# CPJKU/beat_this

Hardware: AMD Instinct MI355X
Metric: audio-seconds processed/sec (higher is better)
Workload: dtype f32 activations, f16x3 products (3 x f16 MFMA on hi+lo operand halves, f32 accumulate); main-layer attention P.V: 2 x, probabilities as fp16 hi parts

## Files before the change

beat_this_amd/_lib.py:

```python
from __future__ import annotations

import ctypes as C
import os
import subprocess

import torch

PKG_DIR = os.path.dirname(os.path.abspath(__file__))
LIB_PATH = os.path.join(PKG_DIR, "libbeat_this_amd.so")
if os.environ.get("BT_DEV") == "1" and os.environ.get("BT_LIB_PATH"):
    LIB_PATH = os.environ["BT_LIB_PATH"]
SOURCES = ["gemm.hip", "gemm2.hip", "gemm3.hip", "gemm_mx8.hip", "attn.hip", "attn2.hip", "fused.hip", "fused2.hip", "qkv_front.hip", "frontend.hip", "logmel.hip",
           "tail.hip", "dbn.hip", "metrics.hip", "loss.hip", "data.hip", "train.hip", "optim.hip", "engine.hip"]
HEADERS = ["common.h", "chain.h", "kernels.h", "attn_x3_loop.inc", "attn_hq2_loop.inc", os.path.join("..", "..", "include", "beat_this_amd.h")]

BT_OK, BT_ERR_ARG, BT_ERR_HIP, BT_ERR_WORKSPACE = 0, -1, -2, -3
ABI_VERSION = 600
PREC_F32, PREC_HALF, PREC_F32X3 = 0, 1, 3
OPT_X3_ATTN_P16, OPT_X3_GEMM_FP8, OPT_WS_GUARD = 1, 2, 3
MAX_LAYERS = 32
PROFILE_CATEGORIES = ["stem", "qkv_gemm", "attn_flash", "out_gemm", "ff1_gemm", "ff2_gemm", "conv_gemm",
                      "linear_gemm", "head", "ff_fused", "attn_freq_fused", "layer_tail"]

GEMM_EPI_STORE, GEMM_EPI_RESID, GEMM_EPI_QKV = 0, 1, 2
GEMM_F_RMS, GEMM_F_BIAS, GEMM_F_GELU, GEMM_F_OUT_F32, GEMM_F_A_F32, GEMM_F_CONV, GEMM_F_ROWMAP = 1, 2, 4, 8, 16, 32, 64


class PairWeights(C.Structure):
    _fields_ = [("dim", C.c_int32), ("heads", C.c_int32), ("w_qkvg", C.c_void_p * 2), ("b_gates", C.c_void_p),
                ("w_out", C.c_void_p * 2), ("w_ff1", C.c_void_p * 2), ("b_ff1", C.c_void_p),
                ("w_ff2", C.c_void_p * 2), ("b_ff2", C.c_void_p),
                ("w_ff_frag", C.c_void_p * 2), ("w_qkv_frag", C.c_void_p),
                ("w_outff_frag", C.c_void_p * 2), ("w_attnff_frag", C.c_void_p * 2),
                ("w_tail_frag", C.c_void_p),
# ... 352 lines not shown
```

beat_this_amd/csrc/engine.hip:

```cpp
#include <algorithm>
#include <cmath>
#include <cstddef>
#include <cstdio>
#include <cstring>
#include <mutex>
#include <string>
#include <vector>

#include "../../include/beat_this_amd.h"
#include "common.h"
#include "kernels.h"


static thread_local std::string g_err;
static int bt_set_error(int code, const std::string& msg) {
  g_err = msg;
  return code;
}
int bt_set_error_external(int code, const char* msg) { return bt_set_error(code, msg); }

namespace prof {
struct Rec { int cat; hipEvent_t a, b; };
struct State { bool on = false; std::vector<Rec> recs; };
struct Scope {
// ... 9 lines not shown
};
}

struct FwdGraph { int B, T, prec; void* ws; hipGraphExec_t exec; unsigned long stamp; };

struct bt_engine {
  bt_model_desc d;
  prof::State prof;
  std::mutex mu;
  std::vector<FwdGraph> graphs;
  unsigned long graph_clock = 0;
  hipStream_t cap_stream = nullptr;
  std::vector<int> warm;
  int x3_attn_p16 = 1;
  int x3_gemm_fp8 = 0;
  int ws_guard = 0;
};
enum { CAT_STEM = 0, CAT_QKV, CAT_ATTN_FLASH, CAT_OUT, CAT_FF1, CAT_FF2, CAT_CONV, CAT_LINEAR,
       CAT_HEAD, CAT_FF_FUSED, CAT_ATTN_FREQ_FUSED, CAT_LAYER_TAIL, CAT_COUNT };

namespace {

inline size_t align_up(size_t v, size_t a) { return (v + a - 1) / a * a; }

struct Workspace {
  float* xa; float* xb; float* xm; float* gates; void* xmb;
  void* qkv; void* ao; void* hid;
  void* qf; void* kf; void* vf; float* gates_h; int nbp;
  float* ssq[2];
  int* status;
// ... 120 lines not shown
  bool qkv8;
  bool out8;
  bool ff8;
  bool next8;
  bool tail;
  bool shadow_dead;
};

enum { LAYERS_GENERIC, LAYERS_FRAG_HALF, LAYERS_FRAG_X3 };

struct Route {
  bool x3;
  int fp;
  int gp, wp;
  int x3_attn, x3_attn_front;
  bool half_shadow;
  int layers;
  struct Block { PairRoute freq, time; bool conv3; bool x_dead; } blk[3];
  bool lin3, lin_f8;
  struct Layer { PairRoute pair; FragLayer frag; } layer[BT_MAX_LAYERS];
};

#ifndef BT_SKIP_DEAD_STORES
#define BT_SKIP_DEAD_STORES 1
#endif
Route plan_route(const bt_engine& e, int B, int T, int prec, int first, int last, const Workspace& ws) {
  const bt_model_desc& d = e.d;
  const int D = d.transformer_dim;
  Route r;
  r.x3 = prec == BT_PREC_F32X3;
  r.fp = r.x3 ? BT_PREC_F32 : prec;
  r.gp = prec;
  r.wp = r.x3 ? BT_PREC_HALF : prec;
  r.x3_attn = r.x3 ? 4 | ((e.x3_attn_p16 == 1 || e.x3_attn_p16 == 2) ? BT_X3_P16 : 0) : 0;
  r.x3_attn_front = r.x3 ? 4 | (e.x3_attn_p16 >= 2 ? BT_X3_P16 : 0) : 0;
  auto pair = [&](const bt_pair_weights& w) {
    PairRoute p;
    p.ff_fused = w.dim <= 128 && w.w_ff_frag[r.fp];
    p.outff = p.ff_fused && w.w_outff_frag[r.fp] && w.w_attnff_frag[r.fp];
    p.split = r.x3 && w.w_outff_frag_x3 && w.w_attnff_frag_x3;
    p.time_frag = r.x3 ? p.outff && p.split && w.w_qkv_frag_x3 : p.ff_fused && r.fp == BT_PREC_HALF && w.w_qkv_frag;
    return p;
  };

  r.half_shadow = prec == BT_PREC_HALF && D >= 128 && D % 64 == 0;
  const long wide = (long)B * T * d.ff_mult * D;
  bool frag_x3 = r.x3 && D >= 128 && D % 128 == 0 && wide * 4 < 0x7fffffffL;
  for (int l = 0; frag_x3 && l < d.n_layers; ++l)
    frag_x3 = d.layers[l].w_qkvg_x3 && d.layers[l].w_out_x3 && d.layers[l].w_ff1_x3 && d.layers[l].w_ff2_x3;
  const bool frag_half = r.half_shadow && D % 128 == 0 && wide * 2 < 0x7fffffffL;
  r.layers = frag_x3 ? LAYERS_FRAG_X3 : frag_half ? LAYERS_FRAG_HALF : LAYERS_GENERIC;

  const bool lin3_fits = (frag_half || (frag_x3 && d.lin_w_x3)) && gemm3_supported(linear3_params(d, ws, B, T, frag_x3, false));
  for (int blk = 0; blk < 3; ++blk) {
    Route::Block& rb = r.blk[blk];
    rb.freq = pair(d.front[blk][0]);
    rb.time = pair(d.front[blk][1]);
    const Gemm3P cg = conv3_params(d, ws, blk, B, T, frag_x3, blk == 2 && lin3_fits);
    rb.conv3 = d.partial_transformers && rb.time.outff && (frag_x3 ? rb.time.split : frag_half) && cg.N >= 128 && cg.W &&
               gemm3_supported(cg);
    rb.x_dead = BT_SKIP_DEAD_STORES && rb.conv3 && frag_x3;
  }
  r.lin3 = lin3_fits && (!frag_x3 || r.blk[2].conv3);
  r.lin_f8 = r.lin3 && frag_x3 && e.x3_gemm_fp8 >= 2 && d.n_layers > 0 && d.layers[0].w_qkvg_f8;

  for (int l = 0; l < d.n_layers; ++l) {
    const bt_pair_weights& w = d.layers[l];
    FragLayer& f = r.layer[l].frag;
    r.layer[l].pair = pair(w);
    f.qkv8 = l == 0 ? first == 0 && r.lin_f8 : r.layer[l - 1].frag.next8;
    f.out8 = frag_x3 && e.x3_gemm_fp8 >= 2 && w.w_out_f8;
    f.ff8 = frag_x3 && e.x3_gemm_fp8 >= 1 && w.w_ff1_f8 && w.w_ff2_f8;
    f.next8 = frag_x3 && e.x3_gemm_fp8 >= 2 && l + 1 < d.n_layers && d.layers[l + 1].w_qkvg_f8 && w.w_ff2_f8;
    f.tail = frag_half && w.w_tail_frag && layer_tail_supported(D, d.ff_mult * D);
// ... 143 lines not shown
  AttnFragP a;
  memset(&a, 0, sizeof a);
  a.q = ws.qf; a.k = ws.kf; a.v = ws.vf; a.gates = ws.gates_h; a.out = ws.ao; a.heads = H; a.inner = D; a.nbp = ws.nbp;
  attn_rows(a, B, T, 1);
  a.x3 = r.x3_attn; a.out_f32 = f.out8 ? 2 : 0; a.status = status; a.fix_mask = ws.fix_mask;
  LAUNCH_CAT(CAT_ATTN_FLASH, s, launch_attn_frag(a, s), r.x3 ? "attention (hi + lo)" : "attention");
  if (f.tail) {
    LayerTailP t;
    t.x = ws.xm; t.M = M; t.C = D; t.hidden = HID; t.ao = ws.ao; t.wfrag = pw.w_tail_frag; t.b1 = pw.b_ff1; t.b2 = pw.b_ff2;
    t.xb = ws.xmb; t.ssq_out = ws.ssq[0];
    LAUNCH_CAT(CAT_LAYER_TAIL, s, launch_layer_tail(t, s), "layer tail (out-projection + feed-forward)");
    return BT_OK;
  }
  memset(&g, 0, sizeof g);
  g.A = ws.ao; g.lda = D; g.M = M; g.K = D; g.W = w(pw.w_out, pw.w_out_x3, pw.w_out_f8, f.out8); g.N = D; g.epi = G3_RESID;
  g.x3 = r.x3 | (f.out8 ? G3_X3_F8 : 0) | (f.ff8 ? G3_X3_OUT_F8 : 0); g.status = status;
  g.x = ws.xm; g.ldx = D; g.xb = ws.xmb; g.ssq_out = ws.ssq[1];
  LAUNCH_CAT(CAT_OUT, s, launch_gemm3(g, s), r.x3 ? "out-proj gemm (hi + lo)" : "out-proj gemm");
  memset(&g, 0, sizeof g);
  g.A = ws.xmb; g.lda = D; g.M = M; g.K = D; g.W = w(pw.w_ff1, pw.w_ff1_x3, pw.w_ff1_f8, f.ff8); g.N = HID; g.epi = G3_FF1;
  g.x3 = r.x3 | (f.ff8 ? G3_X3_F8 | G3_X3_OUT_F8 : 0); g.status = status;
  g.bias = pw.b_ff1; g.ssq_in = ws.ssq[1]; g.ssq_parts = parts; g.out = ws.hid; g.ldo = HID;
  LAUNCH_CAT(CAT_FF1, s, launch_gemm3(g, s), r.x3 ? "ff1 gemm (hi + lo)" : "ff1 gemm");
  memset(&g, 0, sizeof g);
  g.A = ws.hid; g.lda = HID; g.M = M; g.K = HID; g.W = w(pw.w_ff2, pw.w_ff2_x3, pw.w_ff2_f8, f.ff8); g.N = D; g.epi = G3_RESID;
  g.x3 = r.x3 | (f.ff8 ? G3_X3_F8 : 0) | (f.next8 ? G3_X3_OUT_F8 : 0); g.status = status;
  g.bias = pw.b_ff2; g.x = ws.xm; g.ldx = D; g.xb = f.shadow_dead ? nullptr : ws.xmb; g.ssq_out = f.shadow_dead ? nullptr : ws.ssq[0];
  LAUNCH_CAT(CAT_FF2, s, launch_gemm3(g, s), r.x3 ? "ff2 gemm (hi + lo)" : "ff2 gemm");
  return BT_OK;
}

int frontend(prof::State* pf, const bt_model_desc& d, const Route& r, const float* spect, const Workspace& ws, int B, int T,
             hipStream_t s) {
  const StemP sp = stem_params(d, spect, front_x(ws, 0), B, T);
  LAUNCH_CAT(CAT_STEM, s, launch_stem(sp, s), "stem");
  for (int blk = 0; blk < 3; ++blk) {
    const Route::Block& rb = r.blk[blk];
    float* x = front_x(ws, blk);
    if (d.partial_transformers) {
      if (int rc = freq_half(pf, d.front[blk][0], rb.freq, r, d.rope, x, B, T, 32 >> blk, s)) return rc;
      if (int rc = time_half(pf, d.front[blk][1], rb.time, r, d.rope, x, ws, B, T, 32 >> blk, rb.conv3 ? ws.hid : nullptr, rb.x_dead, s))
        return rc;
    }
    if (rb.conv3) {
      const Gemm3P g = conv3_params(d, ws, blk, B, T, r.layers == LAYERS_FRAG_X3, blk == 2 && r.lin3);
      LAUNCH_CAT(CAT_CONV, s, launch_gemm3(g, s), "frontend conv gemm");
    } else {
      const GemmP g = conv_params(d, blk, r.wp, x, front_x(ws, blk + 1), B, T, !(blk == 2 && r.lin3));
      LAUNCH_CAT(CAT_CONV, s, launch_gemm(g, r.gp, s), "frontend conv gemm");
    }
  }
  if (r.lin3) {
    const Gemm3P g = linear3_params(d, ws, B, T, r.layers == LAYERS_FRAG_X3, r.lin_f8);
    LAUNCH_CAT(CAT_LINEAR, s, launch_gemm3(g, s), "frontend linear gemm");
    return BT_OK;
  }
  const GemmP g = linear_params(d, r.wp, front_x(ws, 3), ws.xm, r.half_shadow ? ws.xmb : nullptr,
                                r.layers == LAYERS_FRAG_HALF ? ws.ssq[0] : nullptr, B, T);
  LAUNCH_CAT(CAT_LINEAR, s, launch_gemm(g, r.gp, s), "frontend linear gemm");
  if (r.layers == LAYERS_FRAG_X3)
    LAUNCH_CAT(CAT_LINEAR, s, launch_shadow_ssq(ws.xm, ws.xmb, ws.ssq[0], (long)B * T, d.transformer_dim, s, 1), "hl32 shadow of the residual stream");
  return BT_OK;
}

}

extern "C" {

// ... 25 lines not shown
  e->warm.clear();
}
void bt_engine_destroy(bt_engine* e) {
  if (!e) return;
  for (auto& r : e->prof.recs) { (void)hipEventDestroy(r.a); (void)hipEventDestroy(r.b); }
  drop_graphs(e);
  if (e->cap_stream) (void)hipStreamDestroy(e->cap_stream);
  delete e;
}

int bt_engine_set_option(bt_engine* e, int option, int value) {
  if (!e) return bt_set_error(BT_ERR_ARG, "null argument");
  std::lock_guard<std::mutex> lock(e->mu);
  if (option == BT_OPT_X3_ATTN_P16 && value >= 0 && value <= 3) { if (e->x3_attn_p16 != value) drop_graphs(e); e->x3_attn_p16 = value; return BT_OK; }
  if (option == BT_OPT_X3_GEMM_FP8 && value >= 0 && value <= 2) { if (e->x3_gemm_fp8 != value) drop_graphs(e); e->x3_gemm_fp8 = value; return BT_OK; }
  if (option == BT_OPT_WS_GUARD && value >= 0 && value % 256 == 0) { if (e->ws_guard != value) drop_graphs(e); e->ws_guard = value; return BT_OK; }
  return bt_set_error(BT_ERR_ARG, "unknown engine option / value");
}
int bt_engine_get_option(const bt_engine* e, int option, int* value) {
  if (!e || !value) return bt_set_error(BT_ERR_ARG, "null argument");
  if (option == BT_OPT_X3_ATTN_P16) { *value = e->x3_attn_p16; return BT_OK; }
  if (option == BT_OPT_X3_GEMM_FP8) { *value = e->x3_gemm_fp8; return BT_OK; }
  if (option == BT_OPT_WS_GUARD) { *value = e->ws_guard; return BT_OK; }
  return bt_set_error(BT_ERR_ARG, "unknown engine option");
}

size_t bt_workspace_bytes(const bt_engine* e, int B, int T, int prec) {
  if (!e || B <= 0 || T <= 0) return 0;
  return carve(nullptr, B, T, e->d.transformer_dim, e->d.ff_mult, prec, (size_t)e->ws_guard).total;
}

int bt_workspace_regions(const bt_engine* e, int B, int T, int prec, int64_t* begin_end, int max) {
  if (!e || B <= 0 || T <= 0 || max < 0 || (max > 0 && !begin_end)) return bt_set_error(BT_ERR_ARG, "bad argument to bt_workspace_regions");
  if (prec != BT_PREC_F32 && prec != BT_PREC_HALF && prec != BT_PREC_F32X3) return bt_set_error(BT_ERR_ARG, "unknown precision");
  std::vector<int64_t> r;
  carve(nullptr, B, T, e->d.transformer_dim, e->d.ff_mult, prec, (size_t)e->ws_guard, &r);
  const int n = (int)(r.size() / 2);
// ... 565 lines not shown
```

beat_this_amd/csrc/fused2.hip:

```cpp
#include <cstdlib>
#include <type_traits>

#include "chain.h"
#include "kernels.h"

namespace {


typedef __amdgpu_buffer_rsrc_t rsrc_t;
typedef __attribute__((address_space(3))) void* lptr_t;
DEVI unsigned pk2_hf(float a, float b) {
  const hfx2 t = {(hf)a, (hf)b};
  return __builtin_bit_cast(unsigned, t);
}

#ifdef BT_DEV
__device__ long long* g_f2_dbg = nullptr;
#define F2_DBG g_f2_dbg
#define F2_ABL(p) ((p).abl)
#else
#define F2_DBG ((long long*)nullptr)
#define F2_ABL(p) 0
#endif

// ... 321 lines not shown
  const long long t_ff = dbg ? clock64() : 0;
  ff_tail<T, C>(ws, 1 + 2 * H, xn, b1s, p.b2, xrow, nullptr, ok, lane, g);
  if (dbg && lane == 0) {
    long long* d = dbg + ((long)blockIdx.x * 4 + wave) * 6;
    d[0] = t_ring - t_in; d[1] = t_ff - t_ring; d[2] = clock64() - t_ff; d[3] = ws.t_wait; d[4] = ws.t_bar; d[5] = 0;
  }
}

template <typename T>
int launch_outff_t(const FusedOutFFP& p, hipStream_t s) {
  dim3 grid((unsigned)((p.M + 127) / 128)), block(256);
  if constexpr (std::is_same<T, hl>::value) {
    if (p.shadow_only) {
      if (!p.xb) return -2;
      switch (p.C) {
        case 64: hipLaunchKernelGGL((outff_fused_kernel<T, 64, false>), grid, block, 0, s, p); break;
        case 128: hipLaunchKernelGGL((outff_fused_kernel<T, 128, false>), grid, block, 0, s, p); break;
        default: return -2;
      }
      return (int)hipGetLastError();
    }
  } else if (p.shadow_only) {
    return -2;
  }
  switch (p.C) {
    case 32: hipLaunchKernelGGL((outff_fused_kernel<T, 32>), grid, block, 0, s, p); break;
    case 64: hipLaunchKernelGGL((outff_fused_kernel<T, 64>), grid, block, 0, s, p); break;
    case 128: hipLaunchKernelGGL((outff_fused_kernel<T, 128>), grid, block, 0, s, p); break;
    default: return -2;
  }
// ... 39 lines not shown
```

beat_this_amd/csrc/gemm3.hip:

```cpp
#include <cstdlib>

#include "common.h"
#include "kernels.h"

struct G3CfgS { static constexpr int BM = 128, BN = 128, BK = 32, WGM = 2, WGN = 2, NST = 3, OCC = 3; };
struct G3CfgB { static constexpr int BM = 256, BN = 256, BK = 64, WGM = 2, WGN = 4, NST = 2, OCC = 1; };
struct G3CfgT { static constexpr int BM = 192, BN = 256, BK = 64, WGM = 2, WGN = 4, NST = 2, OCC = 1; };
struct G3CfgSX { static constexpr int BM = 128, BN = 128, BK = 64, WGM = 2, WGN = 2, NST = 2, OCC = 2; };
struct G3CfgBX { static constexpr int BM = 256, BN = 256, BK = 64, WGM = 2, WGN = 4, NST = 2, OCC = 1; };
struct G3CfgTX { static constexpr int BM = 192, BN = 256, BK = 64, WGM = 2, WGN = 4, NST = 2, OCC = 1; };
struct G3CfgMX { static constexpr int BM = 256, BN = 128, BK = 32, WGM = 2, WGN = 2, NST = 3, OCC = 2; };
struct G3CfgHX { static constexpr int BM = 64, BN = 128, BK = 64, WGM = 2, WGN = 2, NST = 3, OCC = 2; };

#ifndef X3_NSPLIT
#define X3_NSPLIT 2
#endif

namespace {

typedef G3CfgS CfgS;
typedef G3CfgB CfgB;

constexpr unsigned OOB = 0x80000000u;

#ifndef BT_NT_STORE
#define BT_NT_STORE 1
#endif
#if BT_NT_STORE
#define ST_STREAM(ptr, val) __builtin_nontemporal_store((val), (ptr))
#else
#define ST_STREAM(ptr, val) (*(ptr) = (val))
#endif

typedef __amdgpu_buffer_rsrc_t rsrc_t;
typedef __attribute__((address_space(3))) void* lptr_t;
typedef __attribute__((ext_vector_type(4))) unsigned int u32x4;
typedef __attribute__((ext_vector_type(2))) unsigned int u32x2;

DEVI unsigned pk2(float a, float b) {
  const hfx2 t = {(hf)a, (hf)b};
  return __builtin_bit_cast(unsigned, t);
// ... 531 lines not shown
    const int r4 = lane >> 4, cp = lane & 15;
    const unsigned ldx = (unsigned)p.ldx;
    const unsigned off_lane = (unsigned)(row0 + r4) * ldx + (unsigned)nb0;
    unsigned colq[4];
#pragma unroll
    for (int q = 0; q < 4; ++q) colq[q] = (unsigned)((cp ^ (4 * q + r4)) << 2);
    const int rows_left = p.M - row0 - r4;
    if (p.gelu) {
#pragma unroll
      for (int a = 0; a < FB; ++a)
#pragma unroll
        for (int b = 0; b < TB; ++b)
#pragma unroll
          for (int r = 0; r < 16; ++r) acc[a][b][r] = X3 ? gelu_erf(acc[a][b][r]) : gelu_tanh(acc[a][b][r]);
    }
#pragma unroll
    for (int b = 0; b < TB; ++b) {
      f32x4 xv[8];
#pragma unroll
      for (int ps = 0; ps < 8; ++ps) {
        const unsigned off = off_lane + (unsigned)(32 * b + 4 * ps) * ldx + colq[ps & 3];
        xv[ps] = (32 * b + 4 * ps < rows_left && !p.no_resid && p.x) ? *reinterpret_cast<const f32x4*>(p.x + off)
                                                               : f32x4{0.f, 0.f, 0.f, 0.f};
      }
#pragma unroll
      for (int a = 0; a < FB; ++a)
#pragma unroll
        for (int q = 0; q < 4; ++q)
          *reinterpret_cast<f32x4*>(wst + lr * 256 + (((8 * a + 2 * q + g) ^ (lr & 15)) << 4)) =
              f32x4{acc[a][b][4 * q], acc[a][b][4 * q + 1], acc[a][b][4 * q + 2], acc[a][b][4 * q + 3]};
#pragma unroll
      for (int ps = 0; ps < 8; ++ps) {
        const int r = ps * 4 + r4;
        const unsigned off = off_lane + (unsigned)(32 * b + 4 * ps) * ldx + colq[ps & 3];
        const bool ok = 32 * b + 4 * ps < rows_left;
        f32x4 v = *reinterpret_cast<const f32x4*>(wst + r * 256 + (cp << 4));
#pragma unroll
        for (int i = 0; i < 4; ++i) v[i] += xv[ps][i];
        if (ok) {
          if (p.x) *reinterpret_cast<f32x4*>(p.x + off) = v;
          if constexpr (X3) {
            if (xb) {
              const unsigned f = (unsigned)nb0 + colq[ps & 3];
              unsigned wh[2], wl[2];
              split2(v[0], v[1], wh[0], wl[0], amax);
              split2(v[2], v[3], wh[1], wl[1], amax);
              hf* d = xb + (2u * off - (f & 31u));
              *reinterpret_cast<u32x2*>(d) = u32x2{wh[0], wh[1]};
              if (p.x3 & G3_X3_OUT_F8) {
                char* gb = reinterpret_cast<char*>(d) - (f & 31u);
                *reinterpret_cast<unsigned*>(gb + 64) = pk4_f8(v[0], v[1], v[2], v[3]);
                *reinterpret_cast<unsigned*>(gb + 96) = lo4_f8(v[0], v[1], v[2], v[3], wh[0], wh[1]);
              } else {
                *reinterpret_cast<u32x2*>(d + 32) = u32x2{wl[0], wl[1]};
              }
            }
          } else {
            if (xb) *reinterpret_cast<u32x2*>(xb + off) = u32x2{pk2(v[0], v[1]), pk2(v[2], v[3])};
          }
        }
        if (p.ssq_out) {
          float ssq = ok ? fmaf(v[0], v[0], fmaf(v[1], v[1], fmaf(v[2], v[2], v[3] * v[3]))) : 0.f;
#pragma unroll
          for (int o = 8; o > 0; o >>= 1) ssq += __shfl_xor(ssq, o);
          if (ok && cp == 0) p.ssq_out[(unsigned)(n0 / 64 + wn) * (unsigned)p.M + (unsigned)(row0 + 32 * b + r)] = ssq;
        }
      }
    }
    }
  } else {
    constexpr int BLK_E = X3 ? 2048 : 1024;
    if (kind < 2) {
      hf* dst = reinterpret_cast<hf*>(kind == 0 ? p.qf : p.kf);
#pragma unroll
      for (int b = 0; b < TB; ++b) {
        if (tseq[b] >= p.n_seq) continue;
        const f32x4 (&cs)[4] = csv[b];
#pragma unroll
        for (int a = 0; a < FB; ++a) {
          const int head = (n0 - kind * p.inner + wn * 64 + a * 32) >> 5;
          hf* blk = dst + (((long)tseq[b] * p.heads + head) * p.nbp + tblk[b]) * BLK_E;
#pragma unroll
// ... 127 lines not shown
  const int force = (p.x3 & 15) == 2 ? 1 : (p.x3 & 15) == 3 ? 0 : force_big;
  const bool forced_small = (p.x3 & 15) == 4 || (p.x3 & 15) == 5;
  const long tiles192 = ((long)p.M + 191) / 192 * (p.N / 256);
  const bool fills = !p.x3 || tiles192 >= 160;
  const bool big = big_ok && !forced_small && (force == 1 || (force != 0 && p.epi == G3_RESID && p.K >= 1024 && p.M >= 4096 && fills) ||
                              (force != 0 && p.x3 && X3_BIG_FF1 && p.epi == G3_FF1 && p.M >= 4096));
  auto cost = [&](int bm) { const long t = ((long)p.M + bm - 1) / bm * (p.N / 256); return (t + 255) / 256 * bm; };
  const bool rows192 = big && p.epi == G3_RESID && force != 1 && cost(192) < cost(256);
  const long mx_tiles = ((long)p.M + 255) / 256 * ((p.N + 127) / 128);
  const bool f8 = (p.x3 & G3_X3_F8) != 0;
  const bool mx = p.x3 && !f8 && p.epi != G3_QKV && !big && !rows192 && force != 0 &&
                  ((p.x3 & 15) == 4 || (X3_MX && mx_tiles >= 512 && p.M >= 20000));
  const long sx_tiles = ((long)p.M + 127) / 128 * ((p.N + 127) / 128);
  const bool hx = p.x3 && p.epi == G3_RESID && !big && !rows192 && !mx &&
                  ((p.x3 & 15) == 5 || ((p.x3 & 15) <= 1 && force_big < 0 && (sx_tiles < 256 || (p.K < 1024 && p.M < 20000))));
  if (p.x3) {
#ifdef BT_DEV
    if (abl == 8 && p.epi == G3_FF1) { launch_cfg<G3_FF1, G3CfgSX, true, 8>(p, s); return (int)hipGetLastError(); }
    if (abl == 1 || abl == 4) {
      const bool b = big || rows192;
      if (p.epi == G3_FF1) { if (abl == 1) { if (b) launch_cfg<G3_FF1, G3CfgBX, true, 1>(p, s); else launch_cfg<G3_FF1, G3CfgSX, true, 1>(p, s); }
                             else { if (b) launch_cfg<G3_FF1, G3CfgBX, true, 4>(p, s); else launch_cfg<G3_FF1, G3CfgSX, true, 4>(p, s); } }
      else if (p.epi == G3_RESID) { if (abl == 1) { if (b) launch_cfg<G3_RESID, G3CfgBX, true, 1>(p, s); else launch_cfg<G3_RESID, G3CfgSX, true, 1>(p, s); }
                                    else { if (b) launch_cfg<G3_RESID, G3CfgBX, true, 4>(p, s); else launch_cfg<G3_RESID, G3CfgSX, true, 4>(p, s); } }
      else { if (abl == 1) launch_cfg<G3_QKV, G3CfgSX, true, 1>(p, s); else launch_cfg<G3_QKV, G3CfgSX, true, 4>(p, s); }
      return (int)hipGetLastError();
    }
#endif
    if (f8) {
      if (p.epi == G3_QKV) launch_cfg<G3_QKV, G3CfgSX, 2>(p, s);
      else if (p.epi == G3_FF1) { if (big) launch_cfg<G3_FF1, G3CfgBX, 2>(p, s); else launch_cfg<G3_FF1, G3CfgSX, 2>(p, s); }
      else if (hx) launch_cfg<G3_RESID, G3CfgHX, 2>(p, s);
      else if (rows192) launch_cfg<G3_RESID, G3CfgTX, 2>(p, s);
      else if (big) launch_cfg<G3_RESID, G3CfgBX, 2>(p, s);
      else launch_cfg<G3_RESID, G3CfgSX, 2>(p, s);
      return (int)hipGetLastError();
    }
    switch (p.epi) {
      case G3_FF1:
        if (mx) launch_cfg<G3_FF1, G3CfgMX, true>(p, s);
        else if (big) launch_cfg<G3_FF1, G3CfgBX, true>(p, s); else launch_cfg<G3_FF1, G3CfgSX, true>(p, s);
        break;
      case G3_RESID:
        if (mx) launch_cfg<G3_RESID, G3CfgMX, true>(p, s);
        else if (hx) launch_cfg<G3_RESID, G3CfgHX, true>(p, s);
        else if (rows192) launch_cfg<G3_RESID, G3CfgTX, true>(p, s);
        else if (big) launch_cfg<G3_RESID, G3CfgBX, true>(p, s);
        else launch_cfg<G3_RESID, G3CfgSX, true>(p, s);
        break;
      case G3_QKV: launch_cfg<G3_QKV, G3CfgSX, true>(p, s); break;
      default: return -1;
    }
    return (int)hipGetLastError();
  }
  switch (p.epi) {
    case G3_FF1:
      if (big) launch_cfg<G3_FF1, CfgB>(p, s);
#ifdef BT_DEV
      else if (abl == 8) launch_cfg<G3_FF1, CfgS, false, 8>(p, s);
// ... 18 lines not shown
```

beat_this_amd/csrc/kernels.h:

```cpp
#pragma once
#include <hip/hip_runtime.h>
#include <stdint.h>

#ifndef BT_PREC_F32
#define BT_PREC_F32 0
#define BT_PREC_HALF 1
#endif
#ifndef BT_PREC_F32X3
#define BT_PREC_F32X3 3
#endif

enum {
  GEMM_EPI_STORE = 0,
  GEMM_EPI_RESID = 1,
  GEMM_EPI_QKV = 2
};
enum {
  GEMM_F_RMS = 1,
  GEMM_F_BIAS = 2,
  GEMM_F_GELU = 4,
  GEMM_F_OUT_F32 = 8,
  GEMM_F_A_F32 = 16,
  GEMM_F_CONV = 32,
  GEMM_F_ROWMAP = 64
// ... 28 lines not shown
  const void* W; int N;
  int epi;
  const float* bias;
  const float* ssq_in; int ssq_parts;
  void* out; long ldo;
  float* x; long ldx; void* xb;
  float* ssq_out;
  int n_seq, L, nblk, nbp, heads, inner;
  const float* rope; void* qf; void* kf; void* vf; float* gates; const float* b_gates;
  int no_resid;
  int gelu;
  int conv_C2, conv_T, conv_F;
  int x3;
  int* status;
};
enum { G3_X3_F8 = 0x100, G3_X3_OUT_F8 = 0x200 };
bool gemm3_supported(const Gemm3P& p);
int launch_gemm3(const Gemm3P& p, hipStream_t s);

struct GemmMx8P {
  const void* A; const void* SA;
  const void* W; const void* SW;
  float* out; long ldo;
  int M, N, K;
};
bool gemm_mx8_supported(const GemmMx8P& p);
int launch_gemm_mx8(const GemmMx8P& p, hipStream_t s);

struct AttnP {
  const void* qkv;
  long ld;
// ... 121 lines not shown
```

beat_this_amd/pack.py:

```python
from __future__ import annotations

import collections
import ctypes as C
import math
import threading

import torch

from . import _lib, tables

LOG2E = 1.4426950408889634
BN_EPS = 1e-5


def perm32(w: torch.Tensor) -> torch.Tensor:
    idx = torch.tensor([(r & 3) + 8 * (r >> 2) + 4 * g for g in range(2) for r in range(16)])
    n, k = w.shape
    return w.reshape(n, k // 32, 32)[:, :, idx].reshape(n, k).contiguous()


def fragment_tiles(w: torch.Tensor) -> torch.Tensor:
    r, k = w.shape
    t = w.reshape(r // 32, 32, k // 32, 2, 16)
    return t.permute(0, 2, 3, 1, 4).reshape(r // 32, k // 32, 64, 16)
# ... 79 lines not shown
        d.bn1_shift = self._f32(sd["frontend.stem.bn1d.bias"] - sd["frontend.stem.bn1d.running_mean"] * s1)
        s2 = sd["frontend.stem.bn2d.weight"] / torch.sqrt(sd["frontend.stem.bn2d.running_var"] + BN_EPS)
        d.stem_w = self._f32(sd["frontend.stem.conv2d.weight"].reshape(32, 12) * s2[:, None])
        d.stem_b = self._f32(sd["frontend.stem.bn2d.bias"] - sd["frontend.stem.bn2d.running_mean"] * s2)

        dim = 32
        for i in range(3):
            p = f"frontend.blocks.{i}."
            if d.partial_transformers:
                self._pair(d.front[i][0], sd, p + "partial.attnF.", p + "partial.ffF.", dim)
                self._pair(d.front[i][1], sd, p + "partial.attnT.", p + "partial.ffT.", dim)
            sc = sd[p + "norm.weight"] / torch.sqrt(sd[p + "norm.running_var"] + BN_EPS)
            w = sd[p + "conv2d.weight"] * sc[:, None, None, None]
            w = w.permute(0, 3, 2, 1).reshape(2 * dim, 6 * dim)
            d.conv_w[i][0], d.conv_w[i][1] = self._mat(w)
            if 2 * dim >= 128:
                d.conv_w_x3[i] = self._hl32(w)
            d.conv_b[i] = self._f32(sd[p + "norm.bias"] - sd[p + "norm.running_mean"] * sc)
            dim *= 2
        w = sd["frontend.linear.weight"].view(D, dim, 4).permute(0, 2, 1).reshape(D, 4 * dim)
        d.lin_w[0], d.lin_w[1] = self._mat(w)
        d.lin_w_x3 = self._hl32(w)
        d.lin_b = self._f32(sd["frontend.linear.bias"])
        for l in range(L):
            p = f"transformer_blocks.layers.{l}."
            self._pair(d.layers[l], sd, p + "0.", p + "1.", D, x3=True)
        g = sd["transformer_blocks.norm.gamma"]
        d.head_w = self._f32(sd["task_heads.beat_downbeat_lin.weight"] * g[None, :])
        d.norm_out_g, d.head_w_raw = self._f32(g), self._f32(sd["task_heads.beat_downbeat_lin.weight"])
        hb = sd["task_heads.beat_downbeat_lin.bias"]
        d.head_b[0], d.head_b[1] = float(hb[0]), float(hb[1])
        self._freqs = next(v for k, v in sd.items() if k.endswith("rotary_embed.freqs"))
# ... 180 lines not shown
        self._graphs_ok = True
        self.profiling = False
        self._lock = threading.Lock()
        self.last_fallbacks = 0

    def __del__(self):
        try:
            if getattr(self, "_h", None):
                _lib.lib().bt_engine_destroy(self._h)
                self._h = None
        except Exception:
            pass

    MAX_WORKSPACES = 4
    SHRINK_AFTER = 8
    OPTIONS = {"x3_attn_p16": 1, "x3_gemm_fp8": 2, "ws_guard": 3}

    def set_options(self, opts: dict) -> None:
        for name in opts:
            if name not in self.OPTIONS:
                raise ValueError(f"unknown engine option {name!r} (known: {sorted(self.OPTIONS)})")
        if int(opts.get("x3_gemm_fp8", 0)) > 0:
            undo = self.packed.ensure_hl8()
            if undo is not None:
                self._rebuild_handle(undo)
        for name, value in opts.items():
            _lib.check(_lib.lib().bt_engine_set_option(self._h, self.OPTIONS[name], int(value)))
        self._drop_graphs()

    def _drop_graphs(self) -> None:
        self._graphs = collections.OrderedDict()
# ... 207 lines not shown
```

include/beat_this_amd.h:

```cpp
#ifndef BEAT_THIS_AMD_H
#define BEAT_THIS_AMD_H
#include <stddef.h>
#include <stdint.h>

#ifdef __cplusplus
extern "C" {
#endif

#define BT_OK 0
#define BT_ERR_ARG (-1)
#define BT_ERR_HIP (-2)
#define BT_ERR_WORKSPACE (-3)

#define BT_PREC_F32 0
#define BT_PREC_HALF 1

#define BT_PREC_F32X3 3

#define BT_MAX_LAYERS 32

typedef struct bt_engine bt_engine;

typedef struct {
  int32_t dim, heads;
// ... 52 lines not shown
  const int32_t* mel_len;
  const float* mel_w;
} bt_logmel_tables;

const char* bt_last_error(void);
#define BT_ABI_VERSION 600
int bt_version(void);
int bt_half_is_bf16(void);
void bt_struct_sizes(int32_t* out);

int bt_engine_create(const bt_model_desc* desc, bt_engine** out);
void bt_engine_destroy(bt_engine* e);
#define BT_OPT_X3_ATTN_P16 1
#define BT_OPT_X3_GEMM_FP8 2
#define BT_OPT_WS_GUARD 3
int bt_engine_set_option(bt_engine* e, int option, int value);
int bt_engine_get_option(const bt_engine* e, int option, int* value);
size_t bt_workspace_bytes(const bt_engine* e, int B, int T, int prec);
int bt_workspace_regions(const bt_engine* e, int B, int T, int prec, int64_t* begin_end, int max);

int bt_forward(bt_engine* e, void* stream, int prec, const float* d_spect, int B, int T, void* d_ws,
               size_t ws_bytes, float* d_beat, float* d_downbeat);

int bt_forward_stages(bt_engine* e, void* stream, int prec, int first, int last, const float* d_in, int B, int T, void* d_ws,
                      size_t ws_bytes, float* d_out, float* d_beat, float* d_downbeat);

enum { BT_UNIT_STEM = 0, BT_UNIT_PARTIAL = 1, BT_UNIT_CONV = 2, BT_UNIT_LINEAR = 3, BT_UNIT_ATTN = 4, BT_UNIT_FF = 5, BT_UNIT_NORM = 6,
       BT_UNIT_FRONT_ATTN = 7, BT_UNIT_FRONT_FF = 8 };
int bt_forward_unit(bt_engine* e, void* stream, int prec, int unit, int index, const float* d_in, float* d_out, int B, int T,
                    void* d_ws, size_t ws_bytes);
// ... 227 lines not shown
```

Measured before the change: 62460.

## Stage residual reads via buffer-to-LDS DMA and route narrow conv0 through gemm3

The residual GEMM epilogue now prefetches the residual input rows into LDS with buffer_load_lds DMA, double-buffered per row block, instead of loading them into registers. The shadow hi/lo fp16 stores are merged into one 16-byte store per lane using a DPP lane swap. A new 256x64 tile config lets the first frontend conv (N=64) use the x3 gemm3 path, with hi/lo weights now always packed and an extra outff instantiation for 32 channels. An option restores the old register epilogue. These changes aim to cut epilogue load latency and store count and to bring the narrow conv onto the fused path, at the cost of more LDS traffic and wait-count complexity.

```diff
diff --git a/beat_this_amd/_lib.py b/beat_this_amd/_lib.py
--- a/beat_this_amd/_lib.py
+++ b/beat_this_amd/_lib.py
@@ -17,7 +17,7 @@
 BT_OK, BT_ERR_ARG, BT_ERR_HIP, BT_ERR_WORKSPACE = 0, -1, -2, -3
 ABI_VERSION = 600
 PREC_F32, PREC_HALF, PREC_F32X3 = 0, 1, 3
-OPT_X3_ATTN_P16, OPT_X3_GEMM_FP8, OPT_WS_GUARD = 1, 2, 3
+OPT_X3_ATTN_P16, OPT_X3_GEMM_FP8, OPT_WS_GUARD, OPT_X3_RESID_REG = 1, 2, 3, 4
 MAX_LAYERS = 32
 PROFILE_CATEGORIES = ["stem", "qkv_gemm", "attn_flash", "out_gemm", "ff1_gemm", "ff2_gemm", "conv_gemm",
                       "linear_gemm", "head", "ff_fused", "attn_freq_fused", "layer_tail"]
diff --git a/beat_this_amd/csrc/engine.hip b/beat_this_amd/csrc/engine.hip
--- a/beat_this_amd/csrc/engine.hip
+++ b/beat_this_amd/csrc/engine.hip
@@ -47,6 +47,7 @@
   std::vector<int> warm;
   int x3_attn_p16 = 1;
   int x3_gemm_fp8 = 0;
+  int x3_resid_reg = 0;
   int ws_guard = 0;
 };
 enum { CAT_STEM = 0, CAT_QKV, CAT_ATTN_FLASH, CAT_OUT, CAT_FF1, CAT_FF2, CAT_CONV, CAT_LINEAR,
@@ -197,6 +198,7 @@
   int fp;
   int gp, wp;
   int x3_attn, x3_attn_front;
+  int x3_epi;
   bool half_shadow;
   int layers;
   struct Block { PairRoute freq, time; bool conv3; bool x_dead; } blk[3];
@@ -217,6 +219,7 @@
   r.wp = r.x3 ? BT_PREC_HALF : prec;
   r.x3_attn = r.x3 ? 4 | ((e.x3_attn_p16 == 1 || e.x3_attn_p16 == 2) ? BT_X3_P16 : 0) : 0;
   r.x3_attn_front = r.x3 ? 4 | (e.x3_attn_p16 >= 2 ? BT_X3_P16 : 0) : 0;
+  r.x3_epi = (r.x3 && e.x3_resid_reg) ? G3_X3_REG_EPI : 0;
   auto pair = [&](const bt_pair_weights& w) {
     PairRoute p;
     p.ff_fused = w.dim <= 128 && w.w_ff_frag[r.fp];
@@ -240,7 +243,8 @@
     rb.freq = pair(d.front[blk][0]);
     rb.time = pair(d.front[blk][1]);
     const Gemm3P cg = conv3_params(d, ws, blk, B, T, frag_x3, blk == 2 && lin3_fits);
-    rb.conv3 = d.partial_transformers && rb.time.outff && (frag_x3 ? rb.time.split : frag_half) && cg.N >= 128 && cg.W &&
+    const bool wide_enough = cg.N >= 128 || (BT_CONV0_GEMM3 && frag_x3);
+    rb.conv3 = d.partial_transformers && rb.time.outff && (frag_x3 ? rb.time.split : frag_half) && wide_enough && cg.W &&
                gemm3_supported(cg);
     rb.x_dead = BT_SKIP_DEAD_STORES && rb.conv3 && frag_x3;
   }
@@ -414,7 +418,7 @@
   }
   memset(&g, 0, sizeof g);
   g.A = ws.ao; g.lda = D; g.M = M; g.K = D; g.W = w(pw.w_out, pw.w_out_x3, pw.w_out_f8, f.out8); g.N = D; g.epi = G3_RESID;
-  g.x3 = r.x3 | (f.out8 ? G3_X3_F8 : 0) | (f.ff8 ? G3_X3_OUT_F8 : 0); g.status = status;
+  g.x3 = r.x3 | (f.out8 ? G3_X3_F8 : 0) | (f.ff8 ? G3_X3_OUT_F8 : 0) | r.x3_epi; g.status = status;
   g.x = ws.xm; g.ldx = D; g.xb = ws.xmb; g.ssq_out = ws.ssq[1];
   LAUNCH_CAT(CAT_OUT, s, launch_gemm3(g, s), r.x3 ? "out-proj gemm (hi + lo)" : "out-proj gemm");
   memset(&g, 0, sizeof g);
@@ -424,7 +428,7 @@
   LAUNCH_CAT(CAT_FF1, s, launch_gemm3(g, s), r.x3 ? "ff1 gemm (hi + lo)" : "ff1 gemm");
   memset(&g, 0, sizeof g);
   g.A = ws.hid; g.lda = HID; g.M = M; g.K = HID; g.W = w(pw.w_ff2, pw.w_ff2_x3, pw.w_ff2_f8, f.ff8); g.N = D; g.epi = G3_RESID;
-  g.x3 = r.x3 | (f.ff8 ? G3_X3_F8 : 0) | (f.next8 ? G3_X3_OUT_F8 : 0); g.status = status;
+  g.x3 = r.x3 | (f.ff8 ? G3_X3_F8 : 0) | (f.next8 ? G3_X3_OUT_F8 : 0) | r.x3_epi; g.status = status;
   g.bias = pw.b_ff2; g.x = ws.xm; g.ldx = D; g.xb = f.shadow_dead ? nullptr : ws.xmb; g.ssq_out = f.shadow_dead ? nullptr : ws.ssq[0];
   LAUNCH_CAT(CAT_FF2, s, launch_gemm3(g, s), r.x3 ? "ff2 gemm (hi + lo)" : "ff2 gemm");
   return BT_OK;
@@ -443,7 +447,8 @@
         return rc;
     }
     if (rb.conv3) {
-      const Gemm3P g = conv3_params(d, ws, blk, B, T, r.layers == LAYERS_FRAG_X3, blk == 2 && r.lin3);
+      Gemm3P g = conv3_params(d, ws, blk, B, T, r.layers == LAYERS_FRAG_X3, blk == 2 && r.lin3);
+      if (g.x3) g.x3 |= r.x3_epi;
       LAUNCH_CAT(CAT_CONV, s, launch_gemm3(g, s), "frontend conv gemm");
     } else {
       const GemmP g = conv_params(d, blk, r.wp, x, front_x(ws, blk + 1), B, T, !(blk == 2 && r.lin3));
@@ -451,7 +456,8 @@
     }
   }
   if (r.lin3) {
-    const Gemm3P g = linear3_params(d, ws, B, T, r.layers == LAYERS_FRAG_X3, r.lin_f8);
+    Gemm3P g = linear3_params(d, ws, B, T, r.layers == LAYERS_FRAG_X3, r.lin_f8);
+    if (g.x3) g.x3 |= r.x3_epi;
     LAUNCH_CAT(CAT_LINEAR, s, launch_gemm3(g, s), "frontend linear gemm");
     return BT_OK;
   }
@@ -507,6 +513,7 @@
   std::lock_guard<std::mutex> lock(e->mu);
   if (option == BT_OPT_X3_ATTN_P16 && value >= 0 && value <= 3) { if (e->x3_attn_p16 != value) drop_graphs(e); e->x3_attn_p16 = value; return BT_OK; }
   if (option == BT_OPT_X3_GEMM_FP8 && value >= 0 && value <= 2) { if (e->x3_gemm_fp8 != value) drop_graphs(e); e->x3_gemm_fp8 = value; return BT_OK; }
+  if (option == BT_OPT_X3_RESID_REG && (value == 0 || value == 1)) { if (e->x3_resid_reg != value) drop_graphs(e); e->x3_resid_reg = value; return BT_OK; }
   if (option == BT_OPT_WS_GUARD && value >= 0 && value % 256 == 0) { if (e->ws_guard != value) drop_graphs(e); e->ws_guard = value; return BT_OK; }
   return bt_set_error(BT_ERR_ARG, "unknown engine option / value");
 }
@@ -514,6 +521,7 @@
   if (!e || !value) return bt_set_error(BT_ERR_ARG, "null argument");
   if (option == BT_OPT_X3_ATTN_P16) { *value = e->x3_attn_p16; return BT_OK; }
   if (option == BT_OPT_X3_GEMM_FP8) { *value = e->x3_gemm_fp8; return BT_OK; }
+  if (option == BT_OPT_X3_RESID_REG) { *value = e->x3_resid_reg; return BT_OK; }
   if (option == BT_OPT_WS_GUARD) { *value = e->ws_guard; return BT_OK; }
   return bt_set_error(BT_ERR_ARG, "unknown engine option");
 }
diff --git a/beat_this_amd/csrc/fused2.hip b/beat_this_amd/csrc/fused2.hip
--- a/beat_this_amd/csrc/fused2.hip
+++ b/beat_this_amd/csrc/fused2.hip
@@ -359,6 +359,7 @@
     if (p.shadow_only) {
       if (!p.xb) return -2;
       switch (p.C) {
+        case 32: hipLaunchKernelGGL((outff_fused_kernel<T, 32, false>), grid, block, 0, s, p); break;
         case 64: hipLaunchKernelGGL((outff_fused_kernel<T, 64, false>), grid, block, 0, s, p); break;
         case 128: hipLaunchKernelGGL((outff_fused_kernel<T, 128, false>), grid, block, 0, s, p); break;
         default: return -2;
diff --git a/beat_this_amd/csrc/gemm3.hip b/beat_this_amd/csrc/gemm3.hip
--- a/beat_this_amd/csrc/gemm3.hip
+++ b/beat_this_amd/csrc/gemm3.hip
@@ -11,6 +11,7 @@
 struct G3CfgTX { static constexpr int BM = 192, BN = 256, BK = 64, WGM = 2, WGN = 4, NST = 2, OCC = 1; };
 struct G3CfgMX { static constexpr int BM = 256, BN = 128, BK = 32, WGM = 2, WGN = 2, NST = 3, OCC = 2; };
 struct G3CfgHX { static constexpr int BM = 64, BN = 128, BK = 64, WGM = 2, WGN = 2, NST = 3, OCC = 2; };
+struct G3CfgNX { static constexpr int BM = 256, BN = 64, BK = 32, WGM = 4, WGN = 1, NST = 3, OCC = 2; };
 
 #ifndef X3_NSPLIT
 #define X3_NSPLIT 2
@@ -25,6 +26,12 @@
 
 #ifndef BT_NT_STORE
 #define BT_NT_STORE 1
+#endif
+#ifndef BT_RESID_X_DMA
+#define BT_RESID_X_DMA 1
+#endif
+#ifndef BT_RESID_SHADOW16
+#define BT_RESID_SHADOW16 1
 #endif
 #if BT_NT_STORE
 #define ST_STREAM(ptr, val) __builtin_nontemporal_store((val), (ptr))
@@ -586,6 +593,109 @@
 #pragma unroll
           for (int r = 0; r < 16; ++r) acc[a][b][r] = X3 ? gelu_erf(acc[a][b][r]) : gelu_tanh(acc[a][b][r]);
     }
+    auto store_piece = [&](int b, int ps, f32x4 v) {
+      const int r = ps * 4 + r4;
+      const unsigned off = off_lane + (unsigned)(32 * b + 4 * ps) * ldx + colq[ps & 3];
+      const bool ok = 32 * b + 4 * ps < rows_left;
+      if (ok) {
+        if (p.x) *reinterpret_cast<f32x4*>(p.x + off) = v;
+        if constexpr (X3) {
+          if (xb) {
+            const unsigned f = (unsigned)nb0 + colq[ps & 3];
+            unsigned wh[2], wl[2];
+            split2(v[0], v[1], wh[0], wl[0], amax);
+            split2(v[2], v[3], wh[1], wl[1], amax);
+            hf* d = xb + (2u * off - (f & 31u));
+            if (p.x3 & G3_X3_OUT_F8) {
+              *reinterpret_cast<u32x2*>(d) = u32x2{wh[0], wh[1]};
+              char* gb = reinterpret_cast<char*>(d) - (f & 31u);
+              *reinterpret_cast<unsigned*>(gb + 64) = pk4_f8(v[0], v[1], v[2], v[3]);
+              *reinterpret_cast<unsigned*>(gb + 96) = lo4_f8(v[0], v[1], v[2], v[3], wh[0], wh[1]);
+            } else if (BT_RESID_SHADOW16 && X3 == 1) {
+              const bool odd = ((cp ^ r4) & 1) != 0;
+              const unsigned g0 = (unsigned)__builtin_amdgcn_update_dpp(0, (int)(odd ? wh[0] : wl[0]), 0xB1, 0xf, 0xf, false);
+              const unsigned g1 = (unsigned)__builtin_amdgcn_update_dpp(0, (int)(odd ? wh[1] : wl[1]), 0xB1, 0xf, 0xf, false);
+              *reinterpret_cast<u32x4*>(odd ? d + 28 : d) = u32x4{odd ? g0 : wh[0], odd ? g1 : wh[1], odd ? wl[0] : g0, odd ? wl[1] : g1};
+            } else {
+              *reinterpret_cast<u32x2*>(d) = u32x2{wh[0], wh[1]};
+              *reinterpret_cast<u32x2*>(d + 32) = u32x2{wl[0], wl[1]};
+            }
+          }
+        } else {
+          if (xb) *reinterpret_cast<u32x2*>(xb + off) = u32x2{pk2(v[0], v[1]), pk2(v[2], v[3])};
+        }
+      }
+      if (p.ssq_out) {
+        float ssq = ok ? fmaf(v[0], v[0], fmaf(v[1], v[1], fmaf(v[2], v[2], v[3] * v[3]))) : 0.f;
+#pragma unroll
+        for (int o = 8; o > 0; o >>= 1) ssq += __shfl_xor(ssq, o);
+        if (ok && cp == 0) p.ssq_out[(unsigned)(n0 / 64 + wn) * (unsigned)p.M + (unsigned)(row0 + 32 * b + r)] = ssq;
+      }
+    };
+    constexpr bool XDMA = BT_RESID_X_DMA && X3 == 1 && ABL == 0 && NST * ST_BYTES >= NW * 16384;
+    bool dma_done = false;
+    if constexpr (XDMA) {
+      if (!(p.x3 & G3_X3_REG_EPI)) {
+        dma_done = true;
+        char* wx = smem + wave * 16384;
+        const bool use_x = !p.no_resid && p.x;
+        const int rows_w = p.M - row0 < TB * 32 ? p.M - row0 : TB * 32;
+        const unsigned x_bytes = (use_x && rows_w > 0) ? ((unsigned)(rows_w - 1) * ldx + 64u) * 4u : 0u;
+        const float* xbase = p.x ? p.x + ((long)row0 * p.ldx + nb0) : nullptr;
+        const rsrc_t rX = __builtin_amdgcn_make_buffer_rsrc(const_cast<float*>(xbase), 0, x_bytes, 0x00020000);
+        unsigned voffX[4];
+#pragma unroll
+        for (int q = 0; q < 4; ++q) voffX[q] = ((unsigned)r4 * ldx + colq[q]) * 4u;
+        auto issue_x = [&](int b) {
+          char* ar = wx + (b & 1) * 8192;
+#pragma unroll
+          for (int ps = 0; ps < 8; ++ps)
+            __builtin_amdgcn_raw_ptr_buffer_load_lds(rX, (lptr_t)(ar + ps * 1024), 16, 32 * b + 4 * ps < rows_left ? voffX[ps & 3] : OOB,
+                                                     (int)((unsigned)(32 * b + 4 * ps) * ldx * 4u), 0, 0);
+        };
+        if (use_x) {
+          asm volatile("s_waitcnt vmcnt(0)" ::: "memory");
+          __builtin_amdgcn_sched_barrier(0);
+          issue_x(0);
+          if (TB > 1) issue_x(1);
+        }
+#pragma unroll
+        for (int b = 0; b < TB; ++b) {
+          char* ar = wx + (b & 1) * 8192;
+          if (use_x) {
+            if (b + 1 < TB) asm volatile("s_waitcnt vmcnt(8)" ::: "memory");
+            else asm volatile("s_waitcnt vmcnt(0)" ::: "memory");
+            __builtin_amdgcn_sched_barrier(0);
+          }
+          static_assert(FB == 2, "row = 64 features = 256 B");
+          f32x4 xx[8];
+#pragma unroll
+          for (int c = 0; c < 8; ++c) xx[c] = f32x4{0.f, 0.f, 0.f, 0.f};
+          if (use_x) {
+#pragma unroll
+            for (int c = 0; c < 8; ++c)
+              xx[c] = *reinterpret_cast<const f32x4*>(ar + lr * 256 + (((8 * (c >> 2) + 2 * (c & 3) + g) ^ (lr & 15)) << 4));
+          }
+#pragma unroll
+          for (int c = 0; c < 8; ++c) {
+            const int a = c >> 2, q = c & 3;
+            f32x4 v = f32x4{acc[a][b][4 * q], acc[a][b][4 * q + 1], acc[a][b][4 * q + 2], acc[a][b][4 * q + 3]};
+#pragma unroll
+            for (int i = 0; i < 4; ++i) v[i] += xx[c][i];
+            *reinterpret_cast<f32x4*>(ar + lr * 256 + (((8 * a + 2 * q + g) ^ (lr & 15)) << 4)) = v;
+          }
+#pragma unroll
+          for (int ps = 0; ps < 8; ++ps)
+            store_piece(b, ps, *reinterpret_cast<const f32x4*>(ar + (ps * 4 + r4) * 256 + (cp << 4)));
+          if (b + 2 < TB) {
+            asm volatile("s_waitcnt lgkmcnt(0)" ::: "memory");
+            __builtin_amdgcn_sched_barrier(0);
+            if (use_x) issue_x(b + 2);
+          }
+        }
+      }
+    }
+    if (!dma_done) {
 #pragma unroll
     for (int b = 0; b < TB; ++b) {
       f32x4 xv[8];
@@ -603,41 +713,12 @@
               f32x4{acc[a][b][4 * q], acc[a][b][4 * q + 1], acc[a][b][4 * q + 2], acc[a][b][4 * q + 3]};
 #pragma unroll
       for (int ps = 0; ps < 8; ++ps) {
-        const int r = ps * 4 + r4;
-        const unsigned off = off_lane + (unsigned)(32 * b + 4 * ps) * ldx + colq[ps & 3];
-        const bool ok = 32 * b + 4 * ps < rows_left;
-        f32x4 v = *reinterpret_cast<const f32x4*>(wst + r * 256 + (cp << 4));
+        f32x4 v = *reinterpret_cast<const f32x4*>(wst + (ps * 4 + r4) * 256 + (cp << 4));
 #pragma unroll
         for (int i = 0; i < 4; ++i) v[i] += xv[ps][i];
-        if (ok) {
-          if (p.x) *reinterpret_cast<f32x4*>(p.x + off) = v;
-          if constexpr (X3) {
-            if (xb) {
-              const unsigned f = (unsigned)nb0 + colq[ps & 3];
-              unsigned wh[2], wl[2];
-              split2(v[0], v[1], wh[0], wl[0], amax);
-              split2(v[2], v[3], wh[1], wl[1], amax);
-              hf* d = xb + (2u * off - (f & 31u));
-              *reinterpret_cast<u32x2*>(d) = u32x2{wh[0], wh[1]};
-              if (p.x3 & G3_X3_OUT_F8) {
-                char* gb = reinterpret_cast<char*>(d) - (f & 31u);
-                *reinterpret_cast<unsigned*>(gb + 64) = pk4_f8(v[0], v[1], v[2], v[3]);
-                *reinterpret_cast<unsigned*>(gb + 96) = lo4_f8(v[0], v[1], v[2], v[3], wh[0], wh[1]);
-              } else {
-                *reinterpret_cast<u32x2*>(d + 32) = u32x2{wl[0], wl[1]};
-              }
-            }
-          } else {
-            if (xb) *reinterpret_cast<u32x2*>(xb + off) = u32x2{pk2(v[0], v[1]), pk2(v[2], v[3])};
-          }
-        }
-        if (p.ssq_out) {
-          float ssq = ok ? fmaf(v[0], v[0], fmaf(v[1], v[1], fmaf(v[2], v[2], v[3] * v[3]))) : 0.f;
-#pragma unroll
-          for (int o = 8; o > 0; o >>= 1) ssq += __shfl_xor(ssq, o);
-          if (ok && cp == 0) p.ssq_out[(unsigned)(n0 / 64 + wn) * (unsigned)p.M + (unsigned)(row0 + 32 * b + r)] = ssq;
-        }
-      }
+        store_piece(b, ps, v);
+      }
+    }
     }
     }
   } else {
@@ -795,6 +876,7 @@
   const long sx_tiles = ((long)p.M + 127) / 128 * ((p.N + 127) / 128);
   const bool hx = p.x3 && p.epi == G3_RESID && !big && !rows192 && !mx &&
                   ((p.x3 & 15) == 5 || ((p.x3 & 15) <= 1 && force_big < 0 && (sx_tiles < 256 || (p.K < 1024 && p.M < 20000))));
+  const bool nx = BT_CONV0_GEMM3 && p.x3 && !f8 && p.epi == G3_RESID && p.N == 64 && (p.x3 & 15) <= 1 && force_big < 0;
   if (p.x3) {
 #ifdef BT_DEV
     if (abl == 8 && p.epi == G3_FF1) { launch_cfg<G3_FF1, G3CfgSX, true, 8>(p, s); return (int)hipGetLastError(); }
@@ -823,7 +905,8 @@
         else if (big) launch_cfg<G3_FF1, G3CfgBX, true>(p, s); else launch_cfg<G3_FF1, G3CfgSX, true>(p, s);
         break;
       case G3_RESID:
-        if (mx) launch_cfg<G3_RESID, G3CfgMX, true>(p, s);
+        if (nx) launch_cfg<G3_RESID, G3CfgNX, true>(p, s);
+        else if (mx) launch_cfg<G3_RESID, G3CfgMX, true>(p, s);
         else if (hx) launch_cfg<G3_RESID, G3CfgHX, true>(p, s);
         else if (rows192) launch_cfg<G3_RESID, G3CfgTX, true>(p, s);
         else if (big) launch_cfg<G3_RESID, G3CfgBX, true>(p, s);
diff --git a/beat_this_amd/csrc/kernels.h b/beat_this_amd/csrc/kernels.h
--- a/beat_this_amd/csrc/kernels.h
+++ b/beat_this_amd/csrc/kernels.h
@@ -66,7 +66,10 @@
   int x3;
   int* status;
 };
-enum { G3_X3_F8 = 0x100, G3_X3_OUT_F8 = 0x200 };
+enum { G3_X3_F8 = 0x100, G3_X3_OUT_F8 = 0x200, G3_X3_REG_EPI = 0x400 };
+#ifndef BT_CONV0_GEMM3
+#define BT_CONV0_GEMM3 1
+#endif
 bool gemm3_supported(const Gemm3P& p);
 int launch_gemm3(const Gemm3P& p, hipStream_t s);
 
diff --git a/beat_this_amd/pack.py b/beat_this_amd/pack.py
--- a/beat_this_amd/pack.py
+++ b/beat_this_amd/pack.py
@@ -117,8 +117,7 @@
             w = sd[p + "conv2d.weight"] * sc[:, None, None, None]
             w = w.permute(0, 3, 2, 1).reshape(2 * dim, 6 * dim)
             d.conv_w[i][0], d.conv_w[i][1] = self._mat(w)
-            if 2 * dim >= 128:
-                d.conv_w_x3[i] = self._hl32(w)
+            d.conv_w_x3[i] = self._hl32(w)
             d.conv_b[i] = self._f32(sd[p + "norm.bias"] - sd[p + "norm.running_mean"] * sc)
             dim *= 2
         w = sd["frontend.linear.weight"].view(D, dim, 4).permute(0, 2, 1).reshape(D, 4 * dim)
@@ -329,7 +328,7 @@
 
     MAX_WORKSPACES = 4
     SHRINK_AFTER = 8
-    OPTIONS = {"x3_attn_p16": 1, "x3_gemm_fp8": 2, "ws_guard": 3}
+    OPTIONS = {"x3_attn_p16": 1, "x3_gemm_fp8": 2, "ws_guard": 3, "x3_resid_reg": 4}
 
     def set_options(self, opts: dict) -> None:
         for name in opts:
diff --git a/include/beat_this_amd.h b/include/beat_this_amd.h
--- a/include/beat_this_amd.h
+++ b/include/beat_this_amd.h
@@ -90,6 +90,7 @@
 #define BT_OPT_X3_ATTN_P16 1
 #define BT_OPT_X3_GEMM_FP8 2
 #define BT_OPT_WS_GUARD 3
+#define BT_OPT_X3_RESID_REG 4
 int bt_engine_set_option(bt_engine* e, int option, int value);
 int bt_engine_get_option(const bt_engine* e, int option, int* value);
 size_t bt_workspace_bytes(const bt_engine* e, int B, int T, int prec);
```

Result: no change. 62750, median of 6 (+0.5%).
